# gafniguy/4D-Facial-Avatars

Measured on AMD Instinct MI355X. Metric: rays/sec at 512x512, 64 coarse + 128 fine samples, higher is better.
Workload: dtype f32; 1 GPU; configs[1]: paper-model eval forward, 512x512 frame, 64+128 samples, chunksize 65536, perturb on, expression+latent conditioned, background prior; frames sharded over GPUs

## Files before the change

### 4d-facial-avatars_amd/csrc/nf_mlp_live.hip

```cpp
#include "nf_mlp_paper_net.h"

#define NF_LIVE_ROWS 64
#define NF_LIVE_DIR_B (NF_LIVE_ROWS * 1024)
#define NF_LIVE_META_B (NF_LIVE_DIR_B + NF_LIVE_ROWS * 64)
#define NF_LIVE_WAVE_B (NF_LIVE_META_B + NF_LIVE_ROWS * 16)
#define NF_LIVE_SC1 16

static_assert(NF_LIVE_ROWS == 64 && NF_MLP_NT == 2, "ranks wrap with & 63; 31 left over + 32 appended must fit");

__device__ __forceinline__ __amdgpu_buffer_rsrc_t nf_live_ring(char* ring_v) {
    const uint64_t a = (uint64_t)ring_v;
    const uint64_t s = (uint64_t)(uint32_t)__builtin_amdgcn_readfirstlane((int)(uint32_t)a) |
                       ((uint64_t)(uint32_t)__builtin_amdgcn_readfirstlane((int)(a >> 32)) << 32);
    return __builtin_amdgcn_make_buffer_rsrc(reinterpret_cast<char*>(s), (short)0, NF_LIVE_WAVE_B, 0x00020000);
}
__device__ __forceinline__ void nf_live_store(__amdgpu_buffer_rsrc_t ring, int off_b, f32x4 v) {
    __builtin_amdgcn_raw_buffer_store_b128(__builtin_bit_cast(nf_u32x4, v), ring, off_b, 0, 0);
}
__device__ __forceinline__ f32x4 nf_live_load(__amdgpu_buffer_rsrc_t ring, int off_b) {
    return __builtin_bit_cast(f32x4, __builtin_amdgcn_raw_buffer_load_b128(ring, off_b, 0, NF_LIVE_SC1));
}

template <int NT>
__global__ void __launch_bounds__(64 * NF_MLP_WAVES, 1)
k_paper_mlp_fwd_live(const float* __restrict__ packed, const float* __restrict__ cond_, const float* __restrict__ ro,
                     const float* __restrict__ rd, const float* __restrict__ rd_view, const float* __restrict__ z,
                     int64_t n_points, int S, float* __restrict__ raw, float* __restrict__ scratch) {
    using Net = NfPaperNet;
    __shared__ __attribute__((aligned(16))) f32x4 lds[NF_MLP_WAVES * 16 * NT * 64];
    const int lane = threadIdx.x & 63, wave = threadIdx.x >> 6;
    f32x4* act4 = lds + wave * (16 * NT * 64);
    typedef __attribute__((address_space(1))) f32x4 nf_gf32x4;
    nf_gf32x4* raw_v = (nf_gf32x4*)raw;
    asm volatile("" : "+v"(raw_v));
    int stride_v = (int)gridDim.x;
    asm volatile("" : "+v"(stride_v));
    char* ring_v = reinterpret_cast<char*>(scratch) + ((size_t)blockIdx.x * NF_MLP_WAVES + wave) * NF_LIVE_WAVE_B;
    asm volatile("" : "+v"(ring_v));
    const float* z_v = z;
    const float* rdv_v = rd_view;
    asm volatile("" : "+v"(z_v), "+v"(rdv_v));
    int head_v = 0, tail_v = 0;
    asm volatile("" : "+v"(head_v), "+v"(tail_v));
    int rot_v = (int)blockIdx.x, step_v = ((int)gridDim.x * 5 / 13) | 1;
    if (step_v >= (int)gridDim.x) step_v = 0;
    asm volatile("" : "+v"(rot_v), "+v"(step_v));
#pragma unroll 1
    for (int64_t base = 0;; base += __builtin_amdgcn_readfirstlane(stride_v)) {
        const int64_t blk = base + __builtin_amdgcn_readfirstlane(rot_v);
        {
            const int g_n = __builtin_amdgcn_readfirstlane(stride_v);
            int r = __builtin_amdgcn_readfirstlane(rot_v) + __builtin_amdgcn_readfirstlane(step_v);
            rot_v = r >= g_n ? r - g_n : r;
            asm volatile("" : "+v"(rot_v));
        }
        const int64_t p0 = (blk * NF_MLP_WAVES + wave) * (16 * NT);
        int more_v = p0 < n_points;
        asm volatile("" : "+v"(more_v));
        const bool more = __builtin_amdgcn_readfirstlane(more_v) != 0;
        int opaque0 = 0;
        asm volatile("" : "+s"(opaque0));
        const NfW Wi = nf_w_image(packed + opaque0, Net::PACKED), Ci = nf_w_image(cond_ + opaque0, Net::COND_FLOATS);
        if (more) {
            f32x4 pe[NT][4];
            f32x4 dirf[NT][1];
            nf_net_inputs<NT>(pe, dirf, p0, n_points, S, lane, ro, rd, rdv_v, z_v);
            f32x4 acc[NT][16];
            float sigma_raw[NT];
            nf_paper_net_body<Net, NT, 1, true>(acc, sigma_raw, pe, dirf, Wi, Ci, act4, lane);
            int lane_o = lane;
            asm volatile("" : "+v"(lane_o));
            const int g = lane_o >> 4, c = lane_o & 15;
            const __amdgpu_buffer_rsrc_t ring = nf_live_ring(ring_v);
            unsigned m[NT];
            int S_o = S;
            asm volatile("" : "+v"(S_o));
#pragma unroll
            for (int t = 0; t < NT; ++t) {
                const int64_t p = p0 + 16 * t + c;
                const bool mine = g == 0 && p < n_points;
                const bool live = mine && (!(sigma_raw[t] <= 0.0f) || (p + 1) % S_o == 0);
                m[t] = (unsigned)__builtin_amdgcn_ballot_w64(live) & 0xffffu;
                if (mine && !live) raw_v[p] = (f32x4){0.0f, 0.0f, 0.0f, sigma_raw[t]};
            }
            int rows = __builtin_amdgcn_readfirstlane(head_v);
#pragma unroll
            for (int t = 0; t < NT; ++t) {
                if ((m[t] >> c) & 1u) {
                    const int row = (rows + __builtin_popcount(m[t] & ((1u << c) - 1u))) & (NF_LIVE_ROWS - 1);
                    f32x4 v[16];
#pragma unroll
                    for (int j = 0; j < 16; ++j) v[j] = act4[nf_act_idx4(16 * t + c, 4 * j + g)];
#pragma unroll
                    for (int j = 0; j < 16; ++j) nf_live_store(ring, row * 1024 + (4 * j + g) * 16, v[j]);
                    nf_live_store(ring, NF_LIVE_DIR_B + row * 64 + g * 16, dirf[t][0]);
                    if (g == 0) {
                        const int64_t p = p0 + 16 * t + c;
                        nf_live_store(ring, NF_LIVE_META_B + row * 16,
                                      (f32x4){__int_as_float((int)(uint32_t)p), __int_as_float((int)(p >> 32)), 0.0f, 0.0f});
                    }
                }
                rows += __builtin_popcount(m[t]);
            }
            head_v = rows;
            asm volatile("" : "+v"(head_v));
        }
        asm volatile("" : "+v"(more_v));
        const bool last = __builtin_amdgcn_readfirstlane(more_v) == 0;
        const int head = __builtin_amdgcn_readfirstlane(head_v), tail = __builtin_amdgcn_readfirstlane(tail_v);
        const int cnt = head - tail;
        if (cnt >= 16 * NT || (last && cnt > 0)) {
            const int n_valid = cnt < 16 * NT ? cnt : 16 * NT;
            int lane_o = lane;
            asm volatile("" : "+v"(lane_o));
            const int g = lane_o >> 4, c = lane_o & 15;
            const __amdgpu_buffer_rsrc_t ring = nf_live_ring(ring_v);
            __builtin_amdgcn_fence(__ATOMIC_RELEASE, "workgroup");
            __builtin_amdgcn_s_waitcnt(0x0F70);
            __builtin_amdgcn_fence(__ATOMIC_ACQUIRE, "workgroup");
            f32x4 dirf[NT][1], meta[NT];
#pragma unroll
            for (int t = 0; t < NT; ++t) {
                const int row = (tail + 16 * t + c) & (NF_LIVE_ROWS - 1);
                f32x4 v[16];
#pragma unroll
                for (int j = 0; j < 16; ++j) v[j] = nf_live_load(ring, row * 1024 + (4 * j + g) * 16);
#pragma unroll
                for (int j = 0; j < 16; ++j) act4[nf_act_idx4(16 * t + c, 4 * j + g)] = v[j];
                dirf[t][0] = nf_live_load(ring, NF_LIVE_DIR_B + row * 64 + g * 16);
                meta[t] = nf_live_load(ring, NF_LIVE_META_B + row * 16);
            }
            constexpr int NDIR = 1;
            constexpr unsigned D0 = Net::OFF_D0 / 4;
            NfStream<NT> st;
            nf_load_bias<9>(st.bias, Ci, Net::B_D0, lane);
            nf_load_w16<9>(st.wa, Wi, D0, lane);
            nf_read_b<NT>(st.b0, act4, lane, 0);
            f32x4 acc[NT][16], bj[NT];
            float sigma_raw[NT];
            NF_NET_COLOUR();
            int lane_s = lane;
            asm volatile("" : "+v"(lane_s));
            if ((lane_s >> 4) == 0) {
#pragma unroll
                for (int t = 0; t < NT; ++t) {
                    if (16 * t + (lane_s & 15) < n_valid) {
                        const int64_t p = (int64_t)(uint32_t)__float_as_int(meta[t].x) | ((int64_t)__float_as_int(meta[t].y) << 32);
                        if (p >= 0 && p < n_points) raw_v[p] = (f32x4){acc[t][0].x, acc[t][0].y, acc[t][0].z, sigma_raw[t]};
                    }
                }
            }
            tail_v = tail + n_valid;
            asm volatile("" : "+v"(tail_v));
        }
        asm volatile("" : "+v"(more_v));
        if (__builtin_amdgcn_readfirstlane(more_v) == 0) break;
    }
}

static int64_t nf_live_grid_cap(int max_workgroups) {
    const int64_t cu = nf_cu_count();
    return max_workgroups > 0 && max_workgroups < cu ? max_workgroups : cu;
}

extern "C" size_t nf_paper_mlp_fwd_live_scratch_floats(int max_workgroups) {
    return (size_t)nf_live_grid_cap(max_workgroups) * NF_MLP_WAVES * (NF_LIVE_WAVE_B / 4);
}

extern "C" int nf_paper_mlp_fwd_live(const float* packed, const float* cond, const float* ro, const float* rd, const float* rd_view,
                                     const float* z, int64_t n_rays, int n_samples, float* raw, float* scratch, size_t scratch_floats,
                                     int max_workgroups, nf_stream_t stream) {
    static_assert(NF_MLP_WAVES * 16 * NF_MLP_NT == 128, "nf_mlp_fwd_launch sizes the grid for 128 points per workgroup");
    if (max_workgroups < 0 || !scratch || ((uintptr_t)scratch & 15) || scratch_floats < nf_paper_mlp_fwd_live_scratch_floats(max_workgroups))
        return NF_EINVAL;
    const float* rdv = rd_view ? rd_view : rd;
    return nf_mlp_fwd_launch(NF_FWD_INFER, packed, cond, ro, rd, z, raw, nullptr, n_rays, n_samples, [&](int64_t n_points, unsigned grid) {
        const int64_t cap = nf_live_grid_cap(max_workgroups);
        hipLaunchKernelGGL(k_paper_mlp_fwd_live<NF_MLP_NT>, dim3((unsigned)(grid < cap ? grid : cap)), dim3(64 * NF_MLP_WAVES), 0, nf_s(stream),
                           packed, cond, ro, rd, rdv, z, n_points, n_samples, raw, scratch);
    });
}
```

### 4d-facial-avatars_amd/csrc/nf_mlp_paper_net.h

```cpp
#pragma once
#include "nf_mlp_net_common.h"
#include "nf_mlp_smaller_layout.h"
#include "nf_pack.h"

#define NF_NET_COMMON(F)                                                                                                              \
    F(FRAG) F(NCOND) F(OFF_L0) F(OFF_L1) F(OFF_L2) F(OFF_L3) F(OFF_L4) F(OFF_FEAT) F(OFF_D0) F(OFF_D0E) F(OFF_D1) F(OFF_D2) F(OFF_RGB) \
    F(OFF_WC0) F(OFF_WC3) F(OFF_WCD) F(OFF_BIAS) F(B_L0) F(B_L1) F(B_L2) F(B_L3) F(B_L4) F(B_FEAT) F(B_D0) F(B_D1) F(B_D2) F(B_RGB)     \
    F(B_CVEC) F(B_DVEC) F(COND_FLOATS) F(S_PE) F(S_H0) F(S_H1) F(S_H2) F(S_H3) F(S_H4) F(S_FEAT) F(S_D0) F(S_D1) F(S_D2) F(S_DIRF)     \
    F(S_MASK) F(SAVED_PER_POINT) F(Z_L0) F(Z_L1) F(Z_L2) F(Z_L3) F(Z_L4) F(Z_FEAT) F(Z_D0) F(Z_D1) F(Z_D2) F(DZ_PER_POINT)             \
    F(OFFT_RGB) F(OFFT_D2) F(OFFT_D1) F(OFFT_D0) F(OFFT_FEAT) F(OFFT_L4) F(OFFT_L3) F(OFFT_L2) F(OFFT_L1)                              \
    F(G_L0) F(G_L1) F(G_L2) F(G_L3A) F(G_L3B) F(G_L4) F(G_FEAT) F(G_D0A) F(G_D0B) F(G_D1) F(G_D2) F(G_RGB) F(G_ALPHA)                  \
    F(CS_L0) F(CS_D0) F(CS_RGB) F(SLAB_FLOATS) F(GRAD_PARAM_FLOATS) F(GRAD_FLOATS)

struct NfPaperNet {
#define NF_NET_COPY(X) static constexpr int X = nfl::X;
    NF_NET_COMMON(NF_NET_COPY)
    NF_NET_COPY(OFF_L5) NF_NET_COPY(B_L5) NF_NET_COPY(S_H5) NF_NET_COPY(Z_L5) NF_NET_COPY(OFFT_L5) NF_NET_COPY(G_L5)
#undef NF_NET_COPY
    static constexpr bool HAS_L5 = true, D0_EXPR = false;
    static constexpr int PACKED = nfl::PACKED_FLOATS, PACKED_T = nfl::PACKED_T_FLOATS, NPARAMS = NF_PAPER_NUM_PARAMS;
    static constexpr int N_RELU = (nfl::SAVED_PER_POINT - nfl::S_MASK) / 8;
    static constexpr int D0_COLS = 280;
    static constexpr int MODEL = 0;
};

struct NfSmallerNet {
#define NF_NET_COPY(X) static constexpr int X = nsm::X;
    NF_NET_COMMON(NF_NET_COPY)
    NF_NET_COPY(OFF_WCE) NF_NET_COPY(NEXPR) NF_NET_COPY(PACKED) NF_NET_COPY(PACKED_T) NF_NET_COPY(NPARAMS) NF_NET_COPY(N_RELU)
#undef NF_NET_COPY
    static constexpr bool HAS_L5 = false, D0_EXPR = true;
    static constexpr int D0_COLS = 280 + nsm::NEXPR;
    static constexpr int MODEL = 2;
};
#undef NF_NET_COMMON

template <class Net> constexpr int nf_net_n_xyz = Net::HAS_L5 ? 6 : 5;

enum { NF_R_XYZ0_W = 0, NF_R_XYZ3_W = 6, NF_R_L5_W = 10, NF_R_FEAT_W = 12, NF_R_FEAT_B = 13, NF_R_ALPHA_W = 14, NF_R_ALPHA_B = 15,
       NF_R_DIR0_W = 16, NF_R_DIR0_B = 17, NF_R_DIR1_W = 18, NF_R_DIR2_W = 20, NF_R_RGB_W = 24, NF_R_RGB_B = 25 };
template <class Net>
__host__ __device__ constexpr int nf_net_id(int role) {
    return role >= NF_R_RGB_W ? Net::NPARAMS - 2 + (role - NF_R_RGB_W) : (role >= NF_R_FEAT_W && !Net::HAS_L5 ? role - 2 : role);
}
template <class Net>
__host__ __device__ constexpr int nf_net_role(int id) {
    return id >= Net::NPARAMS - 2 ? NF_R_RGB_W + (id - (Net::NPARAMS - 2)) : (id >= NF_R_L5_W && !Net::HAS_L5 ? id + 2 : id);
}

template <class Net>
static void nf_paper_net_table(std::vector<uint32_t>& t) {
    constexpr int NX = nf_net_n_xyz<Net>;
    auto id = [](int role) { return nf_net_id<Net>(role); };
    t.assign(Net::PACKED, NF_ZERO_CODE);
    auto fill = [&](int off, int nk, int no_tiles, int tensor, int n_out, int n_cols, auto col_of, int alpha_row = -1) {
        nf_fill_frag(t, off, nk, no_tiles, [&](int slot, int n) {
            if (n < n_out) {
                const int col = col_of(slot);
                return col >= 0 ? nf_code(tensor, n, col, n_cols) : NF_ZERO_CODE;
            }
            return n == alpha_row && slot < 256 ? nf_code(id(NF_R_ALPHA_W), 0, slot, 256) : NF_ZERO_CODE;
        });
    };
    auto ident = [](int s) { return s; };
    fill(Net::OFF_L0, 4, 16, NF_R_XYZ0_W, 256, 171, [](int s) { return nfl::pe_slot_to_col(s); });
    fill(Net::OFF_L1, 16, 16, 2, 256, 256, ident);
    fill(Net::OFF_L2, 16, 16, 4, 256, 256, ident);
    fill(Net::OFF_L3, 20, 16, NF_R_XYZ3_W, 256, 427, [](int s) { return s < 64 ? nfl::pe_slot_to_col(s) : 171 + (s - 64); });
    fill(Net::OFF_L4, 16, 16, 8, 256, 256, ident);
    if constexpr (Net::HAS_L5) fill(Net::OFF_L5, 16, 16, NF_R_L5_W, 256, 256, ident);
    fill(Net::OFF_FEAT, 16, 16, id(NF_R_FEAT_W), 256, 256, ident);
    fill(Net::OFF_D0, 17, 9, id(NF_R_DIR0_W), 128, Net::D0_COLS,
         [](int s) {
             if (s < 256) return s;
             const int g = ((s - 256) >> 2) & 3, r = (s - 256) & 3;
             return r < 2 ? 256 + 6 * g + 3 * r : -1;
         },
         128);
    fill(Net::OFF_D0E, 18, 9, id(NF_R_DIR0_W), 128, Net::D0_COLS, [](int s) { return s < 280 ? s : -1; }, 128);
    fill(Net::OFF_D1, 8, 8, id(NF_R_DIR1_W), 128, 128, ident);
    fill(Net::OFF_D2, 8, 8, id(NF_R_DIR2_W), 128, 128, ident);
    fill(Net::OFF_RGB, 8, 1, id(NF_R_RGB_W), 3, 128, ident);
    for (int n = 0; n < 256; ++n)
        for (int k = 0; k < Net::NCOND; ++k) {
            t[Net::OFF_WC0 + n * Net::NCOND + k] = nf_code(NF_R_XYZ0_W, n, 63 + k, 171);
            t[Net::OFF_WC3 + n * Net::NCOND + k] = nf_code(NF_R_XYZ3_W, n, 63 + k, 427);
        }
    for (int n = 0; n < 128; ++n) {
        for (int f = 0; f < 4; ++f)
            for (int sc = 0; sc < 2; ++sc)
                for (int comp = 1; comp < 3; ++comp)
                    t[Net::OFF_WCD + n * 16 + 4 * f + 2 * sc + (comp - 1)] = nf_code(id(NF_R_DIR0_W), n, 256 + 6 * f + 3 * sc + comp, Net::D0_COLS);
        if constexpr (Net::D0_EXPR)
            for (int k = 0; k < Net::NEXPR; ++k) t[Net::OFF_WCE + n * Net::NEXPR + k] = nf_code(id(NF_R_DIR0_W), n, 280 + k, Net::D0_COLS);
    }
    for (int n = 0; n < 256; ++n) {
        for (int l = 0; l < NX; ++l) t[Net::OFF_BIAS + 256 * l + n] = nf_code(2 * l + 1, 0, n, 256);
        t[Net::OFF_BIAS + Net::B_FEAT + n] = nf_code(id(NF_R_FEAT_B), 0, n, 256);
    }
    for (int n = 0; n < 128; ++n) {
        t[Net::OFF_BIAS + Net::B_D0 + n] = nf_code(id(NF_R_DIR0_B), 0, n, 128);
        t[Net::OFF_BIAS + Net::B_D1 + n] = nf_code(id(NF_R_DIR1_W) + 1, 0, n, 128);
        t[Net::OFF_BIAS + Net::B_D2 + n] = nf_code(id(NF_R_DIR2_W) + 1, 0, n, 128);
    }
    t[Net::OFF_BIAS + Net::B_D0 + 128] = nf_code(id(NF_R_ALPHA_B), 0, 0, 1);
    for (int n = 0; n < 3; ++n) t[Net::OFF_BIAS + Net::B_RGB + n] = nf_code(id(NF_R_RGB_B), 0, n, 3);
}

template <class Net>
static inline size_t nf_paper_net_saved_floats(int64_t n_points) {
    return (size_t)Net::SAVED_PER_POINT * (size_t)((n_points + 31) & ~(int64_t)31) + Net::N_RELU * 128;
}

template <class Net, bool DIRS>
__device__ __forceinline__ void nf_paper_net_condition(const float* __restrict__ packed, const float* __restrict__ expr,
                                                       const float* __restrict__ latent, float near_z, float far_z, float* __restrict__ cond) {
    __shared__ float cvec[Net::NCOND];
    __shared__ float dvec[16];
    const int tid = threadIdx.x;
    if (tid < 76) cvec[tid] = nf_div(nf_mul(expr[tid], 1.0f), 3.0f);
    else if (tid < Net::NCOND) cvec[tid] = latent[tid - 76];
    if (tid >= 128 && tid < 144) {
        const int k = tid - 128, f = k >> 2, sc = (k >> 1) & 1, comp = k & 1;
        const float a = nf_mul(comp ? far_z : near_z, exp2f((float)f));
        dvec[k] = DIRS ? (sc ? cosf(a) : sinf(a)) : 0.0f;
    }
    __syncthreads();
    const float* bias = packed + Net::OFF_BIAS;
    for (int i = blockIdx.x * blockDim.x + tid; i < Net::COND_FLOATS; i += gridDim.x * blockDim.x) {
        if (i >= Net::B_CVEC) { cond[i] = i < Net::B_DVEC ? cvec[i - Net::B_CVEC] : dvec[i - Net::B_DVEC]; continue; }
        float v = bias[i];
        if (i < Net::B_L1 || (i >= Net::B_L3 && i < Net::B_L4)) {
            const int n = i < Net::B_L1 ? i : i - Net::B_L3;
            const float* w = packed + (i < Net::B_L1 ? Net::OFF_WC0 : Net::OFF_WC3) + n * Net::NCOND;
            float s = 0.0f;
            for (int k = 0; k < Net::NCOND; ++k) s = fmaf(w[k], cvec[k], s);
            v += s;
        } else if ((DIRS || Net::D0_EXPR) && i >= Net::B_D0 && i < Net::B_D0 + 128) {
            float s = 0.0f;
            if (DIRS) {
                const float* w = packed + Net::OFF_WCD + (i - Net::B_D0) * 16;
                for (int k = 0; k < 16; ++k) s = fmaf(w[k], dvec[k], s);
            }
            if constexpr (Net::D0_EXPR) {
                const float* we = packed + Net::OFF_WCE + (i - Net::B_D0) * Net::NEXPR;
                for (int k = 0; k < Net::NEXPR; ++k) s = fmaf(we[k], cvec[k], s);
            }
            v += s;
        }
        cond[i] = v;
    }
}

template <class Net>
static inline dim3 nf_paper_net_condition_grid() { return dim3((Net::COND_FLOATS + 255) / 256); }

#define NF_NET_L3_PE()                                                                                        \
    do {                                                                                                      \
        NF_NET_PE_B(0); nf_chunk<NT, 16, true>(acc, st.wa, bj, st.bias);                                          \
        nf_load_w16<16>(st.wa, Wi, Net::OFF_L3 / 4 + 4 * 16 * 64, lane);    \
        nf_read_b<NT>(st.b0, act4, lane, 0);                                                                  \
        f32x4 w[16];                                                                                          \
        nf_load_w16<16>(w, Wi, Net::OFF_L3 / 4 + 1 * 16 * 64, lane);                                          \
        NF_NET_PE_B(1); nf_chunk<NT, 16, false>(acc, w, bj, st.bias);                                             \
        nf_load_w16<16>(w, Wi, Net::OFF_L3 / 4 + 2 * 16 * 64, lane);                                          \
        NF_NET_PE_B(2); nf_chunk<NT, 16, false>(acc, w, bj, st.bias);                                             \
        nf_load_w16<16>(w, Wi, Net::OFF_L3 / 4 + 3 * 16 * 64, lane);                                          \
        NF_NET_PE_B(3); nf_chunk<NT, 16, false>(acc, w, bj, st.bias);                                             \
    } while (0)

#define NF_NET_COLOUR()                                                                                                    \
                                \
    {                                                                                                                      \
        f32x4 wd[16];                                                                                                      \
        nf_load_w16<9>(wd, Wi, D0 + 16 * 9 * 64, lane);                      \
        nf_seg_lds<NT, 9, true, false>(acc, st, Wi, D0, 16, act4, lane);                                                   \
        nf_pending_b<NT, false>(bj, st);                                                                                   \
        nf_chunk<NT, 9, false>(acc, st.wb, bj, st.bias);                                                                   \
        if (NDIR == 2) {                                                                                                   \
            nf_load_w16<9>(st.wb, Wi, D0 + 17 * 9 * 64, lane);                                                             \
            _Pragma("unroll") for (int t = 0; t < NT; ++t) bj[t] = dirf[t][0];                                             \
            nf_chunk<NT, 9, false>(acc, wd, bj, st.bias);                                                                  \
        }                                                                                                                  \
        _Pragma("unroll") for (int t = 0; t < NT; ++t) bj[t] = dirf[t][NDIR - 1];                                          \
        if constexpr (NDIR == 2) nf_tail<NT, 9, 8, 8, 1>(acc, st.wb, bj, st, Wi, Net::OFF_D1 / 4, Ci, Net::B_D1, act4, lane); \
        else nf_tail<NT, 9, 8, 8, 1>(acc, wd, bj, st, Wi, Net::OFF_D1 / 4, Ci, Net::B_D1, act4, lane);                      \
        _Pragma("unroll") for (int t = 0; t < NT; ++t) sigma_raw[t] = acc[t][8].x;                                         \
    }                                                                                                                      \
                                                                                           \
    nf_seg_lds<NT, 8, true, true>(acc, st, Wi, Net::OFF_D1 / 4, 8, act4, lane);                                            \
    nf_pending_b<NT, true>(bj, st);                                                                                        \
    nf_tail<NT, 8, 8, 8, 1>(acc, st.wb, bj, st, Wi, Net::OFF_D2 / 4, Ci, Net::B_D2, act4, lane);                           \
    nf_seg_lds<NT, 8, true, true>(acc, st, Wi, Net::OFF_D2 / 4, 8, act4, lane);                                            \
    nf_pending_b<NT, true>(bj, st);                                                                                        \
    nf_tail<NT, 8, 8, 1, 1>(acc, st.wb, bj, st, Wi, Net::OFF_RGB / 4, Ci, Net::B_RGB, act4, lane);                         \
                                                                                                     \
    nf_seg_lds<NT, 1, true, true>(acc, st, Wi, Net::OFF_RGB / 4, 8, act4, lane);                                           \
    nf_pending_b<NT, true>(bj, st);                                                                                        \
    nf_chunk<NT, 1, false>(acc, st.wb, bj, st.bias)

template <class Net, int NT, int NDIR, bool SIGMA = false>
__device__ __forceinline__ void nf_paper_net_body(f32x4 (&acc)[NT][16], float (&sigma_raw)[NT], const f32x4 (&pe)[NT][4],
                                                  const f32x4 (&dirf)[NT][NDIR], const NfW& Wi, const NfW& Ci, f32x4* act4, int lane) {
    constexpr unsigned D0 = (NDIR == 1 ? Net::OFF_D0 : Net::OFF_D0E) / 4;
    NfStream<NT> st;
    f32x4 bj[NT];
#define NF_NET_LAYER256(OFF_, FIRST_, OFF_NEXT_, B_NEXT_, NO_NEXT_, NEXT_B_)                                                \
    nf_seg_lds<NT, 16, FIRST_, true>(acc, st, Wi, OFF_, 16, act4, lane);                                                    \
    nf_pending_b<NT, true>(bj, st);                                                                                         \
    nf_tail<NT, 16, 16, NO_NEXT_, NEXT_B_>(acc, st.wb, bj, st, Wi, OFF_NEXT_, Ci, B_NEXT_, act4, lane)
    NF_NET_PE_LAYER(Net::B_L0, Net::OFF_L0, Net::OFF_L1, Net::B_L1);
    NF_NET_LAYER256(Net::OFF_L1 / 4, true, Net::OFF_L2 / 4, Net::B_L2, 16, 1);
    NF_NET_LAYER256(Net::OFF_L2 / 4, true, Net::OFF_L3 / 4, Net::B_L3, 16, 0);
    NF_NET_L3_PE();
    NF_NET_LAYER256(Net::OFF_L3 / 4 + 4 * 16 * 64, false, Net::OFF_L4 / 4, Net::B_L4, 16, 1);
    if constexpr (Net::HAS_L5) {
        NF_NET_LAYER256(Net::OFF_L4 / 4, true, Net::OFF_L5 / 4, Net::B_L5, 16, 1);
        NF_NET_LAYER256(Net::OFF_L5 / 4, true, Net::OFF_FEAT / 4, Net::B_FEAT, 16, 1);
    } else {
        NF_NET_LAYER256(Net::OFF_L4 / 4, true, Net::OFF_FEAT / 4, Net::B_FEAT, 16, 1);
    }
    if constexpr (SIGMA) {
        NF_NET_LAYER256(Net::OFF_FEAT / 4, true, D0 + 8 * 64, Net::B_D0 + 128, 1, 1);
        f32x4 w8[16];
        w8[0] = st.wa[0];
#pragma unroll
        for (int ch = 1; ch < 16; ++ch) w8[ch] = nf_load_w1(Wi, D0 + (9 * ch + 8) * 64, lane);
#pragma unroll
        for (int ch = 0; ch < 16; ++ch) {
            if (ch == 0) {
#pragma unroll
                for (int t = 0; t < NT; ++t) bj[t] = st.b0[t];
            } else {
                nf_read_b<NT>(bj, act4, lane, ch);
            }
#pragma unroll
            for (int r = 0; r < 4; ++r)
#pragma unroll
                for (int t = 0; t < NT; ++t)
                    acc[t][8] = __builtin_amdgcn_mfma_f32_16x16x4f32(w8[ch][r], bj[t][r], (ch == 0 && r == 0) ? st.bias[0] : acc[t][8], 0, 0, 0);
        }
#pragma unroll
        for (int t = 0; t < NT; ++t) sigma_raw[t] = acc[t][8].x;
        return;
    }
    NF_NET_LAYER256(Net::OFF_FEAT / 4, true, D0, Net::B_D0, 9, 1);
#undef NF_NET_LAYER256
    NF_NET_COLOUR();
}

template <class Net, int NT>
__device__ __forceinline__ void nf_paper_net_fwd_encoded(f32x4* lds, const float* __restrict__ packed, const float* __restrict__ cond,
                                                         const float* __restrict__ x87, int64_t n_points, float* __restrict__ out) {
    const int lane = threadIdx.x & 63, wave = threadIdx.x >> 6;
    const int64_t p0 = ((int64_t)blockIdx.x * NF_MLP_WAVES + wave) * (16 * NT);
    if (p0 >= n_points) return;
    f32x4* act4 = lds + wave * (16 * NT * 64);
    f32x4 pe[NT][4];
    f32x4 dirf[NT][2];
    nf_net_inputs_encoded<NT>(pe, dirf, p0, n_points, lane, x87);
    f32x4 acc[NT][16];
    float sigma_raw[NT];
    const NfW Wi = nf_w_image(packed, Net::PACKED), Ci = nf_w_image(cond, Net::COND_FLOATS);
    nf_paper_net_body<Net, NT, 2>(acc, sigma_raw, pe, dirf, Wi, Ci, act4, lane);
    nf_net_store_raw<NT>(acc, sigma_raw, p0, n_points, lane, out);
}

template <class Condition, class Forward>
static inline int nf_paper_net_forward_encoded(const float* packed, const float* x87, const float* expr76, const float* latent32,
                                               int64_t n_points, float* cond, float* out, Condition condition, Forward forward) {
    if (n_points == 0) return 0;
    if (!packed || !x87 || !expr76 || !latent32 || !cond || !out || n_points < 0) return NF_EINVAL;
    condition();
    const int64_t per_block = (int64_t)NF_MLP_WAVES * 16 * NF_MLP_NT;
    const int64_t grid = (n_points + per_block - 1) / per_block;
    if (grid > 0x7fffffff) return NF_EINVAL;
    forward((unsigned)grid);
    NF_RETURN_LAUNCH();
}

template <class Net, int NT>
__device__ __forceinline__ void nf_paper_net_body_save(f32x4 (&acc)[NT][16], float (&sigma_raw)[NT], const f32x4 (&pe)[NT][4],
                                                       const f32x4 (&dirf)[NT][1], const NfW& Wi, const NfW& Ci, f32x4* act4, int lane,
                                                       float* __restrict__ saved, int64_t p0, int64_t n) {
    static_assert(NT == 2, "the copy schedule below is written for 32-point slabs");
    constexpr int NX = nf_net_n_xyz<Net>;
    const int g = lane >> 4, c = lane & 15;
    auto sec = [&](int s, int width) { return nf_slab_copy(saved, s, width, p0, n); };
#pragma unroll
    for (int t = 0; t < NT; ++t) {
        const int64_t p = p0 + 16 * t + c;
        if (p < n) *reinterpret_cast<f32x4*>(saved + Net::S_DIRF * n + p * 16 + 4 * g) = dirf[t][0];
#pragma unroll
        for (int j = 0; j < 4; ++j) act4[nf_act_idx4(16 * t + c, 4 * j + g)] = pe[t][j];
    }
    {
        const NfSlabCopy cp = sec(Net::S_PE, 64);
#pragma unroll
        for (int k = 0; k < 16 * NT / 4; ++k) nf_copy_rows<16>(act4, cp, k, lane);
    }
    uint64_t m64[NT];
    NfStream<NT> st;
    f32x4 bj[NT];
#define NF_NET_LAYER128(OFF_, NO_, SEC_, MASKL_)                                                                          \
    NfCopyH<32, 4, true> cs{act4, sec(SEC_, 128), lane, 4, {}};                                                            \
    cs.prime();                                                                                                            \
    _Pragma("unroll") for (int t = 0; t < NT; ++t) m64[t] = 0;                                                             \
    nf_seg_lds<NT, NO_, true, true, true>(acc, st, Wi, OFF_, 8, act4, lane, cs, m64);                                      \
    NF_NET_SAVE_PENDING(true, MASKL_, 8)
    NF_NET_PE_LAYER(Net::B_L0, Net::OFF_L0, Net::OFF_L1, Net::B_L1);
    NF_NET_SAVE_LAYER256(Net::OFF_L1 / 4, true, Net::S_H0, 0, Net::OFF_L2 / 4, Net::B_L2, 16, 1);
    NF_NET_SAVE_LAYER256(Net::OFF_L2 / 4, true, Net::S_H1, 1, Net::OFF_L3 / 4, Net::B_L3, 16, 0);
    NF_NET_L3_PE();
    NF_NET_SAVE_LAYER256(Net::OFF_L3 / 4 + 4 * 16 * 64, false, Net::S_H2, 2, Net::OFF_L4 / 4, Net::B_L4, 16, 1);
    if constexpr (Net::HAS_L5) {
        NF_NET_SAVE_LAYER256(Net::OFF_L4 / 4, true, Net::S_H3, 3, Net::OFF_L5 / 4, Net::B_L5, 16, 1);
        NF_NET_SAVE_LAYER256(Net::OFF_L5 / 4, true, Net::S_H4, 4, Net::OFF_FEAT / 4, Net::B_FEAT, 16, 1);
        NF_NET_SAVE_LAYER256(Net::OFF_FEAT / 4, true, Net::S_H5, 5, Net::OFF_D0 / 4, Net::B_D0, 9, 1);
    } else {
        NF_NET_SAVE_LAYER256(Net::OFF_L4 / 4, true, Net::S_H3, 3, Net::OFF_FEAT / 4, Net::B_FEAT, 16, 1);
        NF_NET_SAVE_LAYER256(Net::OFF_FEAT / 4, true, Net::S_H4, 4, Net::OFF_D0 / 4, Net::B_D0, 9, 1);
    }
    {
        f32x4 wd[16];
        nf_load_w16<9>(wd, Wi, Net::OFF_D0 / 4 + 16 * 9 * 64, lane);
        NfCopyH<64, 4, false> cs{act4, sec(Net::S_FEAT, 256), lane, 8, {}};
        cs.prime();
        nf_seg_lds<NT, 9, true, false, false>(acc, st, Wi, Net::OFF_D0 / 4, 16, act4, lane, cs, m64);
        NF_NET_SAVE_PENDING(false, -1, 16);
        nf_chunk<NT, 9, false>(acc, st.wb, bj, st.bias);
#pragma unroll
        for (int t = 0; t < NT; ++t) bj[t] = dirf[t][0];
        nf_tail<NT, 9, 8, 8, 1>(acc, wd, bj, st, Wi, Net::OFF_D1 / 4, Ci, Net::B_D1, act4, lane);
#pragma unroll
        for (int t = 0; t < NT; ++t) sigma_raw[t] = acc[t][8].x;
    }
    {
        NF_NET_LAYER128(Net::OFF_D1 / 4, 8, Net::S_D0, NX);
        nf_tail<NT, 8, 8, 8, 1>(acc, st.wb, bj, st, Wi, Net::OFF_D2 / 4, Ci, Net::B_D2, act4, lane);
    }
    {
        NF_NET_LAYER128(Net::OFF_D2 / 4, 8, Net::S_D1, NX + 1);
        nf_tail<NT, 8, 8, 1, 1>(acc, st.wb, bj, st, Wi, Net::OFF_RGB / 4, Ci, Net::B_RGB, act4, lane);
    }
    {
        NF_NET_LAYER128(Net::OFF_RGB / 4, 1, Net::S_D2, NX + 2);
        nf_chunk<NT, 1, false>(acc, st.wb, bj, st.bias);
    }
#undef NF_NET_LAYER128
}
#undef NF_NET_L3_PE

template <class Net, int NT>
__device__ __forceinline__ void nf_paper_net_fwd_save(f32x4* lds, const float* __restrict__ packed, const float* __restrict__ cond,
                                                      const float* __restrict__ ro, const float* __restrict__ rd,
                                                      const float* __restrict__ rd_view, const float* __restrict__ z, int64_t n_points, int S,
                                                      float* __restrict__ raw, float* __restrict__ saved) {
    const int lane = threadIdx.x & 63, wave = threadIdx.x >> 6;
    const int64_t p0 = ((int64_t)blockIdx.x * NF_MLP_WAVES + wave) * (16 * NT);
    if (p0 >= n_points) return;
    f32x4* act4 = lds + wave * (16 * NT * 64);
    f32x4 pe[NT][4];
    f32x4 dirf[NT][1];
    nf_net_inputs<NT>(pe, dirf, p0, n_points, S, lane, ro, rd, rd_view, z);
    f32x4 acc[NT][16];
    float sigma_raw[NT];
    const NfW Wi = nf_w_image(packed, Net::PACKED), Ci = nf_w_image(cond, Net::COND_FLOATS);
    nf_paper_net_body_save<Net, NT>(acc, sigma_raw, pe, dirf, Wi, Ci, act4, lane, saved, p0, n_points);
    nf_net_store_raw<NT>(acc, sigma_raw, p0, n_points, lane, raw);
}

template <class Fwd, class FwdSave>
static inline int nf_paper_net_launch_fwd(Fwd fwd, FwdSave fwd_save, const float* packed, const float* cond, const float* ro, const float* rd,
                                          const float* rd_view, const float* z, int64_t n_rays, int n_samples, float* raw, float* saved,
                                          nf_stream_t stream) {
    static_assert(NF_MLP_WAVES * 16 * NF_MLP_NT == 128, "nf_mlp_fwd_launch sizes the grid for 128 points per workgroup");
    const float* rdv = rd_view ? rd_view : rd;
    return nf_mlp_fwd_launch(saved ? NF_FWD_TRAIN_F32 : NF_FWD_INFER, packed, cond, ro, rd, z, raw, saved, n_rays, n_samples,
                             [&](int64_t n_points, unsigned grid) {
        if (saved)
            hipLaunchKernelGGL(fwd_save, dim3(grid), dim3(64 * NF_MLP_WAVES), 0, nf_s(stream), packed, cond, ro, rd, rdv, z, n_points,
                               n_samples, raw, saved);
        else
            hipLaunchKernelGGL(fwd, dim3((unsigned)(grid < nf_cu_count() ? grid : nf_cu_count())), dim3(64 * NF_MLP_WAVES), 0, nf_s(stream),
                               packed, cond, ro, rd, rdv, z, n_points, n_samples, raw);
    });
}

template <class Net, int NT>
__device__ __forceinline__ void nf_paper_net_fwd_sigma(f32x4* lds, const float* __restrict__ packed, const float* __restrict__ cond_,
                                                       const float* __restrict__ ro, const float* __restrict__ rd, const float* __restrict__ z,
                                                       int64_t n_points, int S, float* __restrict__ sigma) {
    const int lane = threadIdx.x & 63, wave = threadIdx.x >> 6;
    const int c = lane & 15;
    f32x4* act4 = lds + wave * (16 * NT * 64);
    typedef __attribute__((address_space(1))) float nf_gf32;
    nf_gf32* sigma_v = (nf_gf32*)sigma;
    asm volatile("" : "+v"(sigma_v));
    int stride_v = (int)gridDim.x;
    asm volatile("" : "+v"(stride_v));
    const float* z_v = z;
    asm volatile("" : "+v"(z_v));
#pragma unroll 1
    for (int64_t blk = blockIdx.x;; blk += __builtin_amdgcn_readfirstlane(stride_v)) {
        const int64_t p0 = (blk * NF_MLP_WAVES + wave) * (16 * NT);
        if (p0 >= n_points) break;
        int opaque0 = 0;
        asm volatile("" : "+s"(opaque0));
        const float* W = packed + opaque0;
        const float* cond = cond_ + opaque0;
        f32x4 pe[NT][4];
        f32x4 dirf[NT][1];
        nf_net_inputs<NT>(pe, dirf, p0, n_points, S, lane, ro, rd, rd, z_v);
        f32x4 acc[NT][16];
        float sigma_raw[NT];
        const NfW Wi = nf_w_image(W, Net::PACKED), Ci = nf_w_image(cond, Net::COND_FLOATS);
        nf_paper_net_body<Net, NT, 1, true>(acc, sigma_raw, pe, dirf, Wi, Ci, act4, lane);
        int lane_o = lane;
        asm volatile("" : "+v"(lane_o));
        if ((lane_o >> 4) == 0) {
#pragma unroll
            for (int t = 0; t < NT; ++t) {
                const int64_t p = p0 + 16 * t + c;
                if (p < n_points) sigma_v[p] = sigma_raw[t];
            }
        }
    }
}

template <class Sigma>
static inline int nf_paper_net_launch_sigma(Sigma kernel, const float* packed, const float* cond, const float* ro, const float* rd,
                                            const float* z, int64_t n_rays, int n_samples, float* sigma, nf_stream_t stream) {
    static_assert(NF_MLP_WAVES * 16 * NF_MLP_NT == 128, "nf_mlp_fwd_launch sizes the grid for 128 points per workgroup");
    return nf_mlp_fwd_launch(NF_FWD_INFER, packed, cond, ro, rd, z, sigma, nullptr, n_rays, n_samples, [&](int64_t n_points, unsigned grid) {
        hipLaunchKernelGGL(kernel, dim3((unsigned)(grid < nf_cu_count() ? grid : nf_cu_count())), dim3(64 * NF_MLP_WAVES), 0, nf_s(stream),
                           packed, cond, ro, rd, z, n_points, n_samples, sigma);
    });
}
```

### 4d-facial-avatars_amd/csrc/nf_mlp_stream.h

```cpp
#pragma once
#include "nf_mlp_dev.h"

#define NF_TAIL_LAG 2

template <int NT>
struct NfStream {
    f32x4 wa[16], wb[16];
    f32x4 bias[16];
    f32x4 b0[NT], b1[NT];
    f32x4 bp[NT];
};

__device__ __forceinline__ f32x4 nf_relu_i(f32x4 v) {
    f32x4 o;
#pragma unroll
    for (int r = 0; r < 4; ++r) {
        const int xi = __float_as_int(v[r]);
        o[r] = __int_as_float(xi > 0 ? xi : 0);
    }
    return o;
}

struct NfW {
    __amdgpu_buffer_rsrc_t rsrc;
};
__device__ __forceinline__ NfW nf_w_image(const float* base, int n_floats) {
    NfW w;
    w.rsrc = __builtin_amdgcn_make_buffer_rsrc(const_cast<float*>(base), (short)0, n_floats * 4, 0x00020000);
    return w;
}

template <int NO>
__device__ __forceinline__ void nf_load_w16(f32x4 (&w)[16], const NfW& W, unsigned off4, int lane) {
#pragma unroll
    for (int no = 0; no < NO; ++no)
        w[no] = __builtin_bit_cast(f32x4, __builtin_amdgcn_raw_buffer_load_b128(W.rsrc, lane * 16 + (no & 3) * 1024, (int)(off4 * 16u) + (no >> 2) * 4096, 0));
}

__device__ __forceinline__ f32x4 nf_load_w1(const NfW& W, unsigned off4, int lane) {
    return __builtin_bit_cast(f32x4, __builtin_amdgcn_raw_buffer_load_b128(W.rsrc, lane * 16 + (int)(off4 * 16u), 0, 0));
}

template <int NO>
__device__ __forceinline__ void nf_load_bias(f32x4 (&bias)[16], const NfW& C, unsigned off, int lane) {
    const int g = lane >> 4;
#pragma unroll
    for (int no = 0; no < NO; ++no)
        bias[no] = __builtin_bit_cast(f32x4, __builtin_amdgcn_raw_buffer_load_b128(C.rsrc, g * 16 + no * 64, (int)(off * 4u), 0));
}

template <int NT>
__device__ __forceinline__ void nf_read_b(f32x4 (&b)[NT], const f32x4* act4, int lane, int ni) {
    const int g = lane >> 4, c = lane & 15;
#pragma unroll
    for (int t = 0; t < NT; ++t) b[t] = act4[nf_act_idx4(16 * t + c, 4 * ni + g)];
}

template <int NT, int NO, bool FIRST>
__device__ __forceinline__ void nf_chunk(f32x4 (&acc)[NT][16], const f32x4 (&w)[16], const f32x4 (&b)[NT], const f32x4 (&bias)[16]) {
#pragma unroll
    for (int no = 0; no < NO; ++no)
#pragma unroll
        for (int r = 0; r < 4; ++r)
#pragma unroll
            for (int t = 0; t < NT; ++t)
                acc[t][no] = __builtin_amdgcn_mfma_f32_16x16x4f32(w[no][r], b[t][r], (FIRST && r == 0) ? bias[no] : acc[t][no], 0, 0, 0);
}

#define NF_SGB_N(mask, n)                                                              \
    do {                                                                               \
        if ((n) == 1) __builtin_amdgcn_sched_group_barrier(mask, 1, 0);                \
        else if ((n) == 2) __builtin_amdgcn_sched_group_barrier(mask, 2, 0);           \
        else if ((n) == 3) __builtin_amdgcn_sched_group_barrier(mask, 3, 0);           \
        else if ((n) == 4) __builtin_amdgcn_sched_group_barrier(mask, 4, 0);           \
        else if ((n) == 5) __builtin_amdgcn_sched_group_barrier(mask, 5, 0);           \
        else if ((n) == 6) __builtin_amdgcn_sched_group_barrier(mask, 6, 0);           \
    } while (0)

struct NfNoCopy {
    static constexpr int N = 0;
    __device__ __forceinline__ void stores(int) const {}
    __device__ __forceinline__ void reads(int) {}
};

template <int W4, int PER, bool RELU>
struct NfCopyH {
    const f32x4* act4;
    NfSlabCopy cp;
    int lane, n_step;
    f32x4 cv[PER];
    static constexpr int N = PER;
    __device__ __forceinline__ void prime() {
#pragma unroll
        for (int k = 0; k < PER; ++k) cv[k] = nf_copy_read<W4>(act4, k, lane);
    }
    __device__ __forceinline__ void stores(int step) const {
#pragma unroll
        for (int k = 0; k < PER; ++k) nf_copy_write<W4>(RELU ? nf_relu_i(cv[k]) : cv[k], cp, step * PER + k, lane);
    }
    __device__ __forceinline__ void reads(int step) {
        const int nx = step + 1 < n_step ? step + 1 : step;
#pragma unroll
        for (int k = 0; k < PER; ++k) cv[k] = nf_copy_read<W4>(act4, nx * PER + k, lane);
    }
};

template <int NT>
__device__ __forceinline__ void nf_mask_bits(uint64_t (&m64)[NT], const f32x4 (&b)[NT], int ni) {
#pragma unroll
    for (int t = 0; t < NT; ++t) {
        uint32_t nib = 0u;
#pragma unroll
        for (int r = 0; r < 4; ++r) {
            const uint32_t y = (uint32_t)__float_as_int(b[t][r]);
            nib |= (y < 1u ? y : 1u) << r;
        }
        m64[t] |= (uint64_t)nib << (4 * ni);
    }
}

template <int NT, int NO, bool FIRST, bool RELU_IN, bool MASK, bool ST, bool RD, class Side>
__device__ __forceinline__ void nf_half(f32x4 (&acc)[NT][16], const f32x4 (&w)[16], const f32x4 (&raw)[NT], f32x4 (&wn)[16], f32x4 (&rawn)[NT],
                                        const f32x4 (&bias)[16], const NfW& W, unsigned wsrc, const f32x4* act4, int lane, int ni_next, Side& side,
                                        int step, uint64_t (&m64)[NT], f32x4 (&bp)[NT]) {
    constexpr int NS = ST ? Side::N : 0, NR = RD ? Side::N : 0;
    f32x4 b[NT];
#pragma unroll
    for (int t = 0; t < NT; ++t) b[t] = RELU_IN ? nf_relu_i(raw[t]) : raw[t];
    if (MASK && ST) {
        if (!RD) nf_mask_bits<NT>(m64, bp, ni_next - 2);
        nf_mask_bits<NT>(m64, b, ni_next - 1);
    }
    if (MASK && !ST) {
#pragma unroll
        for (int t = 0; t < NT; ++t) bp[t] = b[t];
    }
    nf_read_b<NT>(rawn, act4, lane, ni_next);
    const Side rows = side;
    if (RD) side.reads(step);
    nf_load_w16<NO>(wn, W, wsrc, lane);
    if (ST) rows.stores(step);
    nf_chunk<NT, NO, FIRST>(acc, w, b, bias);
    NF_SGB_N(0x100, NT + NR);
    if (RELU_IN) __builtin_amdgcn_sched_group_barrier(0x002, 4 * NT, 0);
#pragma unroll
    for (int no = 0; no < NO; ++no) {
        __builtin_amdgcn_sched_group_barrier(0x008, 4 * NT, 0);
        __builtin_amdgcn_sched_group_barrier(0x020, 1, 0);
        NF_SGB_N(0x040, (no + 1) * NS / NO - no * NS / NO);
    }
    __builtin_amdgcn_sched_barrier(0);
}

template <int NT, int NO, bool FIRST, bool RELU_IN, bool MASK, class Side>
__device__ __forceinline__ void nf_seg_lds(f32x4 (&acc)[NT][16], NfStream<NT>& st, const NfW& W, unsigned wsec, int nch, const f32x4* act4,
                                           int lane, Side& side, uint64_t (&m64)[NT]) {
    if (MASK) {
#pragma unroll
        for (int t = 0; t < NT; ++t) st.bp[t] = (f32x4){0.f, 0.f, 0.f, 0.f};
    }
    __builtin_amdgcn_sched_barrier(0);
    nf_half<NT, NO, FIRST, RELU_IN, MASK, true, true>(acc, st.wa, st.b0, st.wb, st.b1, st.bias, W, wsec + NO * 64, act4, lane, 1, side, 0, m64, st.bp);
#pragma unroll 1
    for (int ni = 1; ni < nch - 1; ni += 2) {
        const int step = (ni + 1) >> 1;
        nf_half<NT, NO, false, RELU_IN, MASK, true, false>(acc, st.wb, st.b1, st.wa, st.b0, st.bias, W, wsec + (ni + 1) * NO * 64, act4, lane, ni + 1, side,
                                                           step, m64, st.bp);
        nf_half<NT, NO, false, RELU_IN, MASK, false, true>(acc, st.wa, st.b0, st.wb, st.b1, st.bias, W, wsec + (ni + 2) * NO * 64, act4, lane, ni + 2, side,
                                                           step, m64, st.bp);
    }
}
template <int NT, int NO, bool FIRST, bool RELU_IN>
__device__ __forceinline__ void nf_seg_lds(f32x4 (&acc)[NT][16], NfStream<NT>& st, const NfW& W, unsigned wsec, int nch, const f32x4* act4,
                                           int lane) {
    NfNoCopy none;
    uint64_t unused[NT];
    nf_seg_lds<NT, NO, FIRST, RELU_IN, false>(acc, st, W, wsec, nch, act4, lane, none, unused);
}

template <int NT, bool RELU_IN>
__device__ __forceinline__ void nf_pending_b(f32x4 (&b)[NT], const NfStream<NT>& st) {
#pragma unroll
    for (int t = 0; t < NT; ++t) b[t] = RELU_IN ? nf_relu_i(st.b1[t]) : st.b1[t];
}

template <int NT, int NO, int NO_ST, int NO_NEXT, int NEXT_B>
__device__ __forceinline__ void nf_tail(f32x4 (&acc)[NT][16], const f32x4 (&w)[16], const f32x4 (&b)[NT], NfStream<NT>& st,
                                        const NfW& W, unsigned wnext, const NfW& C, unsigned bias_next, f32x4* act4, int lane) {
    constexpr int LAG = NF_TAIL_LAG;
    constexpr int NL = 2 * NO_NEXT;
    const int g = lane >> 4, c = lane & 15;
    __builtin_amdgcn_sched_barrier(0);
    nf_load_bias<NO_NEXT>(st.bias, C, bias_next, lane);
    nf_load_w16<NO_NEXT>(st.wa, W, wnext, lane);
    f32x4 braw[NT];
#pragma unroll
    for (int no = 0; no < NO + LAG; ++no) {
        if (no < NO) {
#pragma unroll
            for (int r = 0; r < 4; ++r)
#pragma unroll
                for (int t = 0; t < NT; ++t) acc[t][no] = __builtin_amdgcn_mfma_f32_16x16x4f32(w[no][r], b[t][r], acc[t][no], 0, 0, 0);
        }
        if (no >= LAG && no - LAG < NO_ST) {
#pragma unroll
            for (int t = 0; t < NT; ++t) act4[nf_act_idx4(16 * t + c, 4 * (no - LAG) + g)] = acc[t][no - LAG];
        }
        if (no == LAG && NEXT_B != 0) {
#pragma unroll
            for (int t = 0; t < NT; ++t) braw[t] = act4[nf_act_idx4(16 * t + c, g)];
        }
    }
#pragma unroll
    for (int no = 0; no < NO + LAG; ++no) {
        if (no < NO) {
            __builtin_amdgcn_sched_group_barrier(0x008, 4 * NT, 0);
            NF_SGB_N(0x020, (no + 1) * NL / NO - no * NL / NO);
        }
        if (no >= LAG && no - LAG < NO_ST) __builtin_amdgcn_sched_group_barrier(0x200, NT, 0);
        if (no == LAG && NEXT_B != 0) __builtin_amdgcn_sched_group_barrier(0x100, NT, 0);
    }
    __builtin_amdgcn_sched_barrier(0);
    if (NEXT_B != 0) {
#pragma unroll
        for (int t = 0; t < NT; ++t) st.b0[t] = braw[t];
    }
}

template <int NT, int NO, int NO_NEXT, bool MASKED>
__device__ __forceinline__ void nf_tail_dz(f32x4 (&acc)[NT][16], const f32x4 (&w)[16], const f32x4 (&b)[NT], NfStream<NT>& st, const NfW& W,
                                           unsigned wnext, f32x4* act4, int lane, const uint2 (&m)[NT]) {
    constexpr int LAG = NF_TAIL_LAG;
    constexpr int NL = NO_NEXT;
    const int g = lane >> 4, c = lane & 15;
    __builtin_amdgcn_sched_barrier(0);
    if (NO_NEXT > 0) nf_load_w16<(NO_NEXT > 0 ? NO_NEXT : 1)>(st.wa, W, wnext, lane);
    f32x4 braw[NT];
#pragma unroll
    for (int no = 0; no < NO + LAG; ++no) {
        if (no < NO) {
#pragma unroll
            for (int r = 0; r < 4; ++r)
#pragma unroll
                for (int t = 0; t < NT; ++t) acc[t][no] = __builtin_amdgcn_mfma_f32_16x16x4f32(w[no][r], b[t][r], acc[t][no], 0, 0, 0);
        }
        if (no >= LAG) {
            const int q = no - LAG;
#pragma unroll
            for (int t = 0; t < NT; ++t) {
                f32x4 v = acc[t][q];
                if (MASKED) {
                    const uint32_t wd = q < 8 ? m[t].x : m[t].y;
#pragma unroll
                    for (int r = 0; r < 4; ++r) {
                        const int keep = ((int)(wd << (31 - (4 * (q & 7) + r)))) >> 31;
                        v[r] = __int_as_float(__float_as_int(v[r]) & keep);
                    }
                }
                act4[nf_act_idx4(16 * t + c, 4 * q + g)] = v;
            }
        }
        if (no == LAG && NO_NEXT > 0) {
#pragma unroll
            for (int t = 0; t < NT; ++t) braw[t] = act4[nf_act_idx4(16 * t + c, g)];
        }
    }
#pragma unroll
    for (int no = 0; no < NO + LAG; ++no) {
        if (no < NO) {
            __builtin_amdgcn_sched_group_barrier(0x008, 4 * NT, 0);
            NF_SGB_N(0x020, (no + 1) * NL / NO - no * NL / NO);
        }
        if (no >= LAG) {
            __builtin_amdgcn_sched_group_barrier(0x002, (MASKED ? 12 : 4) * NT, 0);
            __builtin_amdgcn_sched_group_barrier(0x200, NT, 0);
        }
        if (no == LAG && NO_NEXT > 0) __builtin_amdgcn_sched_group_barrier(0x100, NT, 0);
    }
    __builtin_amdgcn_sched_barrier(0);
    if (NO_NEXT > 0) {
#pragma unroll
        for (int t = 0; t < NT; ++t) st.b0[t] = braw[t];
    }
}
```

Before: 581,300 rays/s.

## Compute sigma with scalar dot product and skip alpha tile in live colour pass

```diff
diff --git a/4d-facial-avatars_amd/csrc/nf_mlp_live.hip b/4d-facial-avatars_amd/csrc/nf_mlp_live.hip
--- a/4d-facial-avatars_amd/csrc/nf_mlp_live.hip
+++ b/4d-facial-avatars_amd/csrc/nf_mlp_live.hip
@@ -97,7 +97,7 @@
                     if (g == 0) {
                         const int64_t p = p0 + 16 * t + c;
                         nf_live_store(ring, NF_LIVE_META_B + row * 16,
-                                      (f32x4){__int_as_float((int)(uint32_t)p), __int_as_float((int)(p >> 32)), 0.0f, 0.0f});
+                                      (f32x4){__int_as_float((int)(uint32_t)p), __int_as_float((int)(p >> 32)), sigma_raw[t], 0.0f});
                     }
                 }
                 rows += __builtin_popcount(m[t]);
@@ -133,12 +133,12 @@
             constexpr int NDIR = 1;
             constexpr unsigned D0 = Net::OFF_D0 / 4;
             NfStream<NT> st;
-            nf_load_bias<9>(st.bias, Ci, Net::B_D0, lane);
-            nf_load_w16<9>(st.wa, Wi, D0, lane);
+            nf_load_bias<8>(st.bias, Ci, Net::B_D0, lane);
+            nf_load_w16<8>(st.wa, Wi, D0, lane);
             nf_read_b<NT>(st.b0, act4, lane, 0);
             f32x4 acc[NT][16], bj[NT];
             float sigma_raw[NT];
-            NF_NET_COLOUR();
+            NF_NET_COLOUR(false);
             int lane_s = lane;
             asm volatile("" : "+v"(lane_s));
             if ((lane_s >> 4) == 0) {
@@ -146,7 +146,7 @@
                 for (int t = 0; t < NT; ++t) {
                     if (16 * t + (lane_s & 15) < n_valid) {
                         const int64_t p = (int64_t)(uint32_t)__float_as_int(meta[t].x) | ((int64_t)__float_as_int(meta[t].y) << 32);
-                        if (p >= 0 && p < n_points) raw_v[p] = (f32x4){acc[t][0].x, acc[t][0].y, acc[t][0].z, sigma_raw[t]};
+                        if (p >= 0 && p < n_points) raw_v[p] = (f32x4){acc[t][0].x, acc[t][0].y, acc[t][0].z, meta[t].z};
                     }
                 }
             }
diff --git a/4d-facial-avatars_amd/csrc/nf_mlp_paper_net.h b/4d-facial-avatars_amd/csrc/nf_mlp_paper_net.h
--- a/4d-facial-avatars_amd/csrc/nf_mlp_paper_net.h
+++ b/4d-facial-avatars_amd/csrc/nf_mlp_paper_net.h
@@ -169,23 +169,24 @@
         NF_NET_PE_B(3); nf_chunk<NT, 16, false>(acc, w, bj, st.bias);                                             \
     } while (0)
 
-#define NF_NET_COLOUR()                                                                                                    \
-                                \
+#define NF_NET_COLOUR(ALPHA_TILE_)                                                                                         \
+                                                                   \
     {                                                                                                                      \
+        constexpr int ND0 = (ALPHA_TILE_) ? 9 : 8;                                                                         \
         f32x4 wd[16];                                                                                                      \
-        nf_load_w16<9>(wd, Wi, D0 + 16 * 9 * 64, lane);                      \
-        nf_seg_lds<NT, 9, true, false>(acc, st, Wi, D0, 16, act4, lane);                                                   \
+        nf_load_w16<ND0>(wd, Wi, D0 + 16 * 9 * 64, lane);                    \
+        nf_seg_lds<NT, ND0, true, false, 9>(acc, st, Wi, D0, 16, act4, lane);                                              \
         nf_pending_b<NT, false>(bj, st);                                                                                   \
-        nf_chunk<NT, 9, false>(acc, st.wb, bj, st.bias);                                                                   \
+        nf_chunk<NT, ND0, false>(acc, st.wb, bj, st.bias);                                                                 \
         if (NDIR == 2) {                                                                                                   \
-            nf_load_w16<9>(st.wb, Wi, D0 + 17 * 9 * 64, lane);                                                             \
+            nf_load_w16<ND0>(st.wb, Wi, D0 + 17 * 9 * 64, lane);                                                           \
             _Pragma("unroll") for (int t = 0; t < NT; ++t) bj[t] = dirf[t][0];                                             \
-            nf_chunk<NT, 9, false>(acc, wd, bj, st.bias);                                                                  \
+            nf_chunk<NT, ND0, false>(acc, wd, bj, st.bias);                                                                \
         }                                                                                                                  \
         _Pragma("unroll") for (int t = 0; t < NT; ++t) bj[t] = dirf[t][NDIR - 1];                                          \
-        if constexpr (NDIR == 2) nf_tail<NT, 9, 8, 8, 1>(acc, st.wb, bj, st, Wi, Net::OFF_D1 / 4, Ci, Net::B_D1, act4, lane); \
-        else nf_tail<NT, 9, 8, 8, 1>(acc, wd, bj, st, Wi, Net::OFF_D1 / 4, Ci, Net::B_D1, act4, lane);                      \
-        _Pragma("unroll") for (int t = 0; t < NT; ++t) sigma_raw[t] = acc[t][8].x;                                         \
+        if constexpr (NDIR == 2) nf_tail<NT, ND0, 8, 8, 1>(acc, st.wb, bj, st, Wi, Net::OFF_D1 / 4, Ci, Net::B_D1, act4, lane); \
+        else nf_tail<NT, ND0, 8, 8, 1>(acc, wd, bj, st, Wi, Net::OFF_D1 / 4, Ci, Net::B_D1, act4, lane);                    \
+        if constexpr (ALPHA_TILE_) { _Pragma("unroll") for (int t = 0; t < NT; ++t) sigma_raw[t] = acc[t][8].x; }          \
     }                                                                                                                      \
                                                                                            \
     nf_seg_lds<NT, 8, true, true>(acc, st, Wi, Net::OFF_D1 / 4, 8, act4, lane);                                            \
@@ -221,32 +222,17 @@
         NF_NET_LAYER256(Net::OFF_L4 / 4, true, Net::OFF_FEAT / 4, Net::B_FEAT, 16, 1);
     }
     if constexpr (SIGMA) {
-        NF_NET_LAYER256(Net::OFF_FEAT / 4, true, D0 + 8 * 64, Net::B_D0 + 128, 1, 1);
-        f32x4 w8[16];
-        w8[0] = st.wa[0];
-#pragma unroll
-        for (int ch = 1; ch < 16; ++ch) w8[ch] = nf_load_w1(Wi, D0 + (9 * ch + 8) * 64, lane);
-#pragma unroll
-        for (int ch = 0; ch < 16; ++ch) {
-            if (ch == 0) {
-#pragma unroll
-                for (int t = 0; t < NT; ++t) bj[t] = st.b0[t];
-            } else {
-                nf_read_b<NT>(bj, act4, lane, ch);
-            }
-#pragma unroll
-            for (int r = 0; r < 4; ++r)
-#pragma unroll
-                for (int t = 0; t < NT; ++t)
-                    acc[t][8] = __builtin_amdgcn_mfma_f32_16x16x4f32(w8[ch][r], bj[t][r], (ch == 0 && r == 0) ? st.bias[0] : acc[t][8], 0, 0, 0);
-        }
-#pragma unroll
-        for (int t = 0; t < NT; ++t) sigma_raw[t] = acc[t][8].x;
+        nf_seg_lds<NT, 16, true, true>(acc, st, Wi, Net::OFF_FEAT / 4, 16, act4, lane);
+        nf_pending_b<NT, true>(bj, st);
+        NfAlpha al;
+        nf_alpha_begin(al, Wi, D0, Ci, Net::B_D0 + 128);
+        nf_tail<NT, 16, 16, 0, 0>(acc, st.wb, bj, st, Wi, 0, Ci, 0, act4, lane);
+        nf_alpha_run<NT>(al, sigma_raw, Wi, D0, act4, lane);
         return;
     }
     NF_NET_LAYER256(Net::OFF_FEAT / 4, true, D0, Net::B_D0, 9, 1);
 #undef NF_NET_LAYER256
-    NF_NET_COLOUR();
+    NF_NET_COLOUR(true);
 }
 
 template <class Net, int NT>
diff --git a/4d-facial-avatars_amd/csrc/nf_mlp_stream.h b/4d-facial-avatars_amd/csrc/nf_mlp_stream.h
--- a/4d-facial-avatars_amd/csrc/nf_mlp_stream.h
+++ b/4d-facial-avatars_amd/csrc/nf_mlp_stream.h
@@ -37,10 +37,6 @@
         w[no] = __builtin_bit_cast(f32x4, __builtin_amdgcn_raw_buffer_load_b128(W.rsrc, lane * 16 + (no & 3) * 1024, (int)(off4 * 16u) + (no >> 2) * 4096, 0));
 }
 
-__device__ __forceinline__ f32x4 nf_load_w1(const NfW& W, unsigned off4, int lane) {
-    return __builtin_bit_cast(f32x4, __builtin_amdgcn_raw_buffer_load_b128(W.rsrc, lane * 16 + (int)(off4 * 16u), 0, 0));
-}
-
 template <int NO>
 __device__ __forceinline__ void nf_load_bias(f32x4 (&bias)[16], const NfW& C, unsigned off, int lane) {
     const int g = lane >> 4;
@@ -54,6 +50,51 @@
     const int g = lane >> 4, c = lane & 15;
 #pragma unroll
     for (int t = 0; t < NT; ++t) b[t] = act4[nf_act_idx4(16 * t + c, 4 * ni + g)];
+}
+
+struct NfAlpha {
+    static constexpr int PRE = 4, RING = 8;
+    float s;
+    f32x4 w[RING][4];
+};
+__device__ __forceinline__ void nf_alpha_load_w(f32x4 (&w)[4], const NfW& W, unsigned off4) {
+#pragma unroll
+    for (int k = 0; k < 4; ++k) w[k] = __builtin_bit_cast(f32x4, __builtin_amdgcn_raw_buffer_load_b128(W.rsrc, k * 256, (int)(off4 * 16u), 0));
+}
+template <int NT>
+__device__ __forceinline__ void nf_alpha_read_x(f32x4 (&x)[4], const f32x4* act4, int lane, int ch) {
+    const int c = lane & 15, p = 16 * ((lane >> 4) % NT) + c;
+#pragma unroll
+    for (int k = 0; k < 4; ++k) x[k] = act4[(p * 64 + 4 * ((ch & 3) ^ (c >> 2)) + (k ^ (c & 3))) + 16 * (ch >> 2)];
+}
+__device__ __forceinline__ void nf_alpha_begin(NfAlpha& al, const NfW& W, unsigned d0, const NfW& C, unsigned bias) {
+    al.s = __builtin_bit_cast(float, __builtin_amdgcn_raw_buffer_load_b32(C.rsrc, 0, (int)(bias * 4u), 0));
+#pragma unroll
+    for (int ch = 0; ch < NfAlpha::PRE; ++ch) nf_alpha_load_w(al.w[ch], W, d0 + (9 * ch + 8) * 64);
+}
+template <int NT>
+__device__ __forceinline__ void nf_alpha_run(NfAlpha& al, float (&sigma_raw)[NT], const NfW& W, unsigned d0, const f32x4* act4, int lane) {
+    int lane_a = lane;
+    asm volatile("" : "+v"(lane_a));
+    f32x4 x[2][4];
+    nf_alpha_read_x<NT>(x[0], act4, lane_a, 0);
+#pragma unroll
+    for (int ch = NfAlpha::PRE; ch < NfAlpha::RING; ++ch) nf_alpha_load_w(al.w[ch], W, d0 + (9 * ch + 8) * 64);
+    __builtin_amdgcn_sched_barrier(0);
+#pragma unroll
+    for (int ch = 0; ch < 16; ++ch) {
+        if (ch + 1 < 16) nf_alpha_read_x<NT>(x[(ch + 1) & 1], act4, lane_a, ch + 1);
+#pragma unroll
+        for (int r = 0; r < 4; ++r)
+#pragma unroll
+            for (int k = 0; k < 4; ++k) al.s = __builtin_fmaf(al.w[ch % NfAlpha::RING][k][r], x[ch & 1][k][r], al.s);
+        if (ch + NfAlpha::RING < 16) nf_alpha_load_w(al.w[ch % NfAlpha::RING], W, d0 + (9 * (ch + NfAlpha::RING) + 8) * 64);
+        asm volatile("" : "+v"(al.s) : : "memory");
+        __builtin_amdgcn_sched_barrier(0);
+    }
+#pragma unroll
+    for (int t = 0; t < NT; ++t)
+        sigma_raw[t] = __int_as_float(__builtin_amdgcn_ds_bpermute((16 * t + (lane_a & 15)) << 2, __float_as_int(al.s)));
 }
 
 template <int NT, int NO, bool FIRST>
@@ -152,7 +193,7 @@
     __builtin_amdgcn_sched_barrier(0);
 }
 
-template <int NT, int NO, bool FIRST, bool RELU_IN, bool MASK, class Side>
+template <int NT, int NO, bool FIRST, bool RELU_IN, bool MASK, class Side, int WS = NO>
 __device__ __forceinline__ void nf_seg_lds(f32x4 (&acc)[NT][16], NfStream<NT>& st, const NfW& W, unsigned wsec, int nch, const f32x4* act4,
                                            int lane, Side& side, uint64_t (&m64)[NT]) {
     if (MASK) {
@@ -160,22 +201,22 @@
         for (int t = 0; t < NT; ++t) st.bp[t] = (f32x4){0.f, 0.f, 0.f, 0.f};
     }
     __builtin_amdgcn_sched_barrier(0);
-    nf_half<NT, NO, FIRST, RELU_IN, MASK, true, true>(acc, st.wa, st.b0, st.wb, st.b1, st.bias, W, wsec + NO * 64, act4, lane, 1, side, 0, m64, st.bp);
+    nf_half<NT, NO, FIRST, RELU_IN, MASK, true, true>(acc, st.wa, st.b0, st.wb, st.b1, st.bias, W, wsec + WS * 64, act4, lane, 1, side, 0, m64, st.bp);
 #pragma unroll 1
     for (int ni = 1; ni < nch - 1; ni += 2) {
         const int step = (ni + 1) >> 1;
-        nf_half<NT, NO, false, RELU_IN, MASK, true, false>(acc, st.wb, st.b1, st.wa, st.b0, st.bias, W, wsec + (ni + 1) * NO * 64, act4, lane, ni + 1, side,
+        nf_half<NT, NO, false, RELU_IN, MASK, true, false>(acc, st.wb, st.b1, st.wa, st.b0, st.bias, W, wsec + (ni + 1) * WS * 64, act4, lane, ni + 1, side,
                                                            step, m64, st.bp);
-        nf_half<NT, NO, false, RELU_IN, MASK, false, true>(acc, st.wa, st.b0, st.wb, st.b1, st.bias, W, wsec + (ni + 2) * NO * 64, act4, lane, ni + 2, side,
+        nf_half<NT, NO, false, RELU_IN, MASK, false, true>(acc, st.wa, st.b0, st.wb, st.b1, st.bias, W, wsec + (ni + 2) * WS * 64, act4, lane, ni + 2, side,
                                                            step, m64, st.bp);
     }
 }
-template <int NT, int NO, bool FIRST, bool RELU_IN>
+template <int NT, int NO, bool FIRST, bool RELU_IN, int WS = NO>
 __device__ __forceinline__ void nf_seg_lds(f32x4 (&acc)[NT][16], NfStream<NT>& st, const NfW& W, unsigned wsec, int nch, const f32x4* act4,
                                            int lane) {
     NfNoCopy none;
     uint64_t unused[NT];
-    nf_seg_lds<NT, NO, FIRST, RELU_IN, false>(acc, st, W, wsec, nch, act4, lane, none, unused);
+    nf_seg_lds<NT, NO, FIRST, RELU_IN, false, NfNoCopy, WS>(acc, st, W, wsec, nch, act4, lane, none, unused);
 }
 
 template <int NT, bool RELU_IN>
```

Result: no change. 583,600 rays/s, median of 6 (+0.4%).
